# GemsLab/H2GCN

Measured on AMD Instinct MI355X. Metric: aggregated edges/sec (1+2-hop SpMM), higher is better.
Workload: dtype f32

## Files before the change

### h2gcn_amd/_capi.py

```python
from __future__ import annotations

import ctypes as C
import os
from pathlib import Path

ABI_VERSION = 5
MAX_HOPS = 8

OK = 0
ERR_INVALID_ARGUMENT = -1
ERR_HIP = -2
ERR_OUT_OF_MEMORY = -3
ERR_BAD_INDEX = -4
ERR_NO_TRANSPOSE = -5
ERR_INTERNAL = -6
ERR_EXCHANGE_TIMEOUT = -7

METRICS_MAX_SETS = 4
XCHG_BLOB_BYTES = 192
XCHG_COPY_ENGINE = 0
XCHG_COPY_KERNEL = 1

DTYPE_F32 = 0
DTYPE_BF16 = 1

PLAN_BUILD_TRANSPOSE = 0x1
PLAN_SKIP_VALIDATION = 0x2
PLAN_HOST_TRANSPOSE = 0x4
PLAN_KEEP_PERMUTATION = 0x8
PLAN_SYMMETRIC_PATTERN = 0x10

EXPORTED_SYMBOLS = (
    "h2gcn_abi_version",
    "h2gcn_last_error",
    "h2gcn_device_count",
    "h2gcn_plan_create",
    "h2gcn_plan_destroy",
    "h2gcn_plan_info",
    "h2gcn_plan_set_values",
    "h2gcn_plan_transpose_sharing",
    "h2gcn_plan_row_constant",
    "h2gcn_plan_device_bytes",
    "h2gcn_spmm_hops_f32",
    "h2gcn_spmm_hops_T_f32",
    "h2gcn_plan_schedule",
    "h2gcn_plan_segment_classes",
    "h2gcn_spmm_workspace_bytes",
    "h2gcn_spmm_hops_opts_f32",
    "h2gcn_spmm_hops_T_opts_f32",
    "h2gcn_spmm_hops_bf16",
    "h2gcn_spmm_hops_T_bf16",
    "h2gcn_sddmm_hops_f32",
    "h2gcn_sddmm_hops_bf16",
    "h2gcn_row_softmax_hops_f32",
    "h2gcn_row_softmax_backward_hops_f32",
    "h2gcn_edge_scores_hops_f32",
    "h2gcn_edge_scores_backward_hops_f32",
    "h2gcn_sddmm_hops_heads_f32",
    "h2gcn_row_softmax_hops_heads_f32",
    "h2gcn_row_softmax_backward_hops_heads_f32",
    "h2gcn_edge_scores_hops_heads_f32",
    "h2gcn_edge_scores_backward_hops_heads_f32",
    "h2gcn_spmm_hops_values_f32",
    "h2gcn_spmm_hops_T_values_f32",
    "h2gcn_ring_scratch_bytes",
    "h2gcn_ring_count",
    "h2gcn_ring_fill",
    "h2gcn_ring_count_rows",
    "h2gcn_ring_fill_rows",
    "h2gcn_hop_normalize",
    "h2gcn_hop_normalize_rows",
    "h2gcn_dropout_dense_small_rows",
    "h2gcn_dropout_dense_workspace_bytes",
    "h2gcn_dropout_dense_f32",
# ... 93 lines not shown
        C.POINTER(C.c_void_p), C.POINTER(C.c_void_p), C.POINTER(C.c_void_p),
        C.POINTER(PlanOpts), C.c_void_p, C.POINTER(C.c_void_p),
    ]
    L.h2gcn_plan_destroy.restype = None
    L.h2gcn_plan_destroy.argtypes = [C.c_void_p]
    L.h2gcn_plan_set_values.restype = C.c_int
    L.h2gcn_plan_set_values.argtypes = [C.c_void_p, C.c_int, C.c_void_p, C.c_void_p]
    L.h2gcn_plan_info.restype = C.c_int
    L.h2gcn_plan_info.argtypes = [
        C.c_void_p, C.c_int, C.POINTER(C.c_int64), C.POINTER(C.c_int64), C.POINTER(C.c_int64),
        C.POINTER(C.c_int64), C.POINTER(C.c_int32),
    ]
    L.h2gcn_spmm_hops_f32.restype = C.c_int
    L.h2gcn_spmm_hops_f32.argtypes = [
        C.c_void_p, C.c_uint32, C.c_void_p, C.c_int64, C.c_int32, C.c_void_p, C.c_int64, C.c_int64, C.c_void_p,
    ]
    L.h2gcn_spmm_hops_T_f32.restype = C.c_int
    L.h2gcn_spmm_hops_T_f32.argtypes = [
        C.c_void_p, C.c_uint32, C.c_void_p, C.c_int64, C.c_int64, C.c_int32, C.c_void_p, C.c_int64, C.c_void_p,
    ]
    L.h2gcn_plan_schedule.restype = C.c_int
    L.h2gcn_plan_schedule.argtypes = [C.c_void_p, C.c_uint32, C.c_int, C.c_int64, C.c_int32] + [C.POINTER(C.c_int32)] * 4
    if hasattr(L, "h2gcn_plan_segment_classes"):
        L.h2gcn_plan_segment_classes.restype = C.c_int
        L.h2gcn_plan_segment_classes.argtypes = [C.c_void_p, C.c_uint32, C.c_int, C.c_int64, C.c_int32] + [C.POINTER(C.c_int64)] * 3
    if hasattr(L, "h2gcn_plan_transpose_sharing"):
        L.h2gcn_plan_transpose_sharing.restype = C.c_int
        L.h2gcn_plan_transpose_sharing.argtypes = [C.c_void_p, C.c_int]
        L.h2gcn_plan_device_bytes.restype = C.c_size_t
        L.h2gcn_plan_device_bytes.argtypes = [C.c_void_p]
    if hasattr(L, "h2gcn_plan_row_constant"):
        L.h2gcn_plan_row_constant.restype = C.c_int
        L.h2gcn_plan_row_constant.argtypes = [C.c_void_p, C.c_int]
    L.h2gcn_spmm_workspace_bytes.restype = C.c_size_t
    L.h2gcn_spmm_workspace_bytes.argtypes = [C.c_void_p, C.c_uint32, C.c_int, C.c_void_p, C.c_int64, C.c_int64, C.c_int32]
    L.h2gcn_spmm_hops_opts_f32.restype = C.c_int
    L.h2gcn_spmm_hops_opts_f32.argtypes = [
        C.c_void_p, C.c_uint32, C.c_void_p, C.c_int64, C.c_int32, C.c_void_p, C.c_int64, C.c_int64,
        C.POINTER(LaunchOpts), C.c_void_p,
    ]
    L.h2gcn_spmm_hops_T_opts_f32.restype = C.c_int
    L.h2gcn_spmm_hops_T_opts_f32.argtypes = [
        C.c_void_p, C.c_uint32, C.c_void_p, C.c_int64, C.c_int64, C.c_int32, C.c_void_p, C.c_int64,
        C.POINTER(LaunchOpts), C.c_void_p,
    ]
    if hasattr(L, "h2gcn_spmm_hops_bf16"):
        L.h2gcn_spmm_hops_bf16.restype = C.c_int
        L.h2gcn_spmm_hops_bf16.argtypes = [
            C.c_void_p, C.c_uint32, C.c_void_p, C.c_int64, C.c_int32, C.c_int, C.c_void_p, C.c_int64, C.c_int64,
            C.POINTER(LaunchOpts), C.c_void_p,
        ]
        L.h2gcn_spmm_hops_T_bf16.restype = C.c_int
        L.h2gcn_spmm_hops_T_bf16.argtypes = [
            C.c_void_p, C.c_uint32, C.c_void_p, C.c_int64, C.c_int64, C.c_int32, C.c_int, C.c_void_p, C.c_int64,
            C.POINTER(LaunchOpts), C.c_void_p,
        ]
    if hasattr(L, "h2gcn_sddmm_hops_f32"):
        sddmm_args = [C.c_void_p, C.c_uint32, C.c_void_p, C.c_int64, C.c_int64, C.c_void_p, C.c_int64, C.c_int32,
                      C.POINTER(C.c_void_p), C.c_void_p]
        L.h2gcn_sddmm_hops_f32.restype = C.c_int
        L.h2gcn_sddmm_hops_f32.argtypes = sddmm_args
        L.h2gcn_sddmm_hops_bf16.restype = C.c_int
        L.h2gcn_sddmm_hops_bf16.argtypes = list(sddmm_args)
    if hasattr(L, "h2gcn_row_softmax_hops_f32"):
        L.h2gcn_row_softmax_hops_f32.restype = C.c_int
        L.h2gcn_row_softmax_hops_f32.argtypes = [C.c_void_p, C.c_uint32, C.POINTER(C.c_void_p), C.POINTER(C.c_void_p), C.c_void_p]
# ... 142 lines not shown
```

### h2gcn_amd/csrc/h2gcn_capi.hip

```cpp
#include <hip/hip_runtime.h>

#include <algorithm>
#include <cstdarg>
#include <cstdlib>
#include <cstdio>
#include <cstring>
#include <deque>
#include <map>
#include <mutex>
#include <memory>
#include <new>
#include <string>
#include <vector>

#include "h2gcn_hip.h"
#include "spmm_kernels.hip.h"

#include "capi_internal.h"

namespace h2gcn {

thread_local std::string g_last_error;

int fail(h2gcn_status st, const char* fmt, ...) {
// ... 11 lines not shown
namespace {

using h2gcn::fail;
using h2gcn::g_last_error;

struct DeviceBuf {
    void* p = nullptr;
    ~DeviceBuf() {
        if (p) (void)hipFree(p);
    }
    DeviceBuf() = default;
    DeviceBuf(DeviceBuf&& o) noexcept : p(o.p) { o.p = nullptr; }
    DeviceBuf(const DeviceBuf&) = delete;
    DeviceBuf& operator=(const DeviceBuf&) = delete;
};

struct HopOperand {
    const int64_t* rowptr = nullptr;
    const int32_t* colidx = nullptr;
    const float* vals = nullptr;
    int64_t nnz = 0;
    std::vector<int64_t> long_rows;
    std::vector<uint8_t> len8;
    int64_t n_short = 0, nnz_short = 0;
    int64_t nnz_long = 0;
    const uint32_t* perm = nullptr;
};

struct LongList {
    DeviceBuf dev;
    int n = 0;
    LongList() = default;
    LongList(LongList&&) noexcept = default;
};

struct ClassLists {
    DeviceBuf short_dev, med_dev;
    int64_t n_short = 0, nnz_short = 0, n_med = 0;
    bool built = false;
    ClassLists() = default;
    ClassLists(ClassLists&&) noexcept = default;
};

}

struct h2gcn_plan {
    int n_hops = 0;
    int64_t n_rows = 0, n_cols = 0;
    int long_threshold = 256;
    int rows_per_wave = 4;
    int variant = 0;
    int slice_cols = 0;
    bool has_transpose = false;
    int device = 0;
    std::vector<HopOperand> fwd;
    std::vector<HopOperand> adj;
    std::deque<DeviceBuf> owned;
    std::vector<int> sharing;
    size_t transpose_bytes = 0;
    std::vector<DeviceBuf> rowval;
    std::vector<char> row_const;
    mutable std::mutex mu;
    mutable std::map<uint64_t, LongList> long_cache;
    mutable std::map<uint64_t, ClassLists> class_cache;
    int short_max = -1;
    double short_min_frac = 0.05;
};

namespace h2gcn {
__global__ void check_colidx_kernel(const int32_t* __restrict__ colidx, int64_t nnz, int64_t n_cols, int* flag) {
    int bad = 0;
    for (int64_t i = (int64_t)blockIdx.x * blockDim.x + threadIdx.x; i < nnz; i += (int64_t)gridDim.x * blockDim.x) {
        const int32_t c = colidx[i];
        bad |= (c < 0) | ((int64_t)c >= n_cols);
    }
    if (bad) atomicOr(flag, 1);
}

__global__ void row_values_kernel(const int64_t* __restrict__ rowptr, const float* __restrict__ vals, int64_t n_rows,
                                  float* __restrict__ rowval, int* flag) {
    const int lane = threadIdx.x & (kWave - 1);
    const int64_t n_waves = ((int64_t)gridDim.x * blockDim.x) / kWave;
    const uint32_t* v = reinterpret_cast<const uint32_t*>(vals);
    int bad = 0;
    for (int64_t r = ((int64_t)blockIdx.x * blockDim.x + threadIdx.x) / kWave; r < n_rows; r += n_waves) {
        const int64_t b = rowptr[r], e = rowptr[r + 1];
        const uint32_t first = b < e ? v[b] : 0u;
        for (int64_t i = b + lane; i < e; i += kWave) bad |= v[i] != first;
        if (lane == 0) reinterpret_cast<uint32_t*>(rowval)[r] = first;
    }
    if (bad) atomicOr(flag, 1);
}

extern template void launch_in_tile_short_rows<32, false, float, float>(const LaunchParams&, const Schedule&, dim3, hipStream_t);
extern template void launch_in_tile_short_rows<16, false, float, float>(const LaunchParams&, const Schedule&, dim3, hipStream_t);
extern template void launch_in_tile_short_rows<32, true, float, float>(const LaunchParams&, const Schedule&, dim3, hipStream_t);
extern template void launch_in_tile_short_rows<16, true, float, float>(const LaunchParams&, const Schedule&, dim3, hipStream_t);
extern template void launch_spmm<false, bf16, float>(const LaunchParams&, const Schedule&, dim3, hipStream_t);
extern template void launch_spmm<false, bf16, bf16>(const LaunchParams&, const Schedule&, dim3, hipStream_t);
extern template void launch_spmm<true, bf16, float>(const LaunchParams&, const Schedule&, dim3, hipStream_t);
extern template void launch_spmm<true, bf16, bf16>(const LaunchParams&, const Schedule&, dim3, hipStream_t);

int transpose_csr_device(int64_t n_rows, int64_t n_cols, int64_t nnz, const int64_t* rowptr, const int32_t* colidx,
                         const float* vals, int64_t** t_rowptr_out, int32_t** t_colidx_out, float** t_vals_out,
                         uint32_t** perm_out_keep, hipStream_t stream, std::string* err);
void permute_values(const uint32_t* perm, const float* vals, int64_t nnz, float* t_vals, hipStream_t stream);
}

namespace {

using h2gcn::HopCsr;
using h2gcn::LaunchParams;
using h2gcn::Schedule;

int transpose_csr_host(int64_t n_rows, int64_t n_cols, const std::vector<int64_t>& rowptr,
                       const std::vector<int32_t>& colidx, const std::vector<float>& vals,
                       std::vector<int64_t>& t_rowptr, std::vector<int32_t>& t_colidx, std::vector<float>& t_vals) {
    const int64_t nnz = rowptr[n_rows];
    t_rowptr.assign(n_cols + 1, 0);
    t_colidx.resize(nnz);
    t_vals.resize(nnz);
    for (int64_t i = 0; i < nnz; ++i) t_rowptr[colidx[i] + 1]++;
    for (int64_t c = 0; c < n_cols; ++c) t_rowptr[c + 1] += t_rowptr[c];
    std::vector<int64_t> cursor(t_rowptr.begin(), t_rowptr.end() - 1);
// ... 139 lines not shown
    auto it = plan->long_cache.find(key);
    if (it == plan->long_cache.end()) {
        const std::vector<HopOperand>& ops = adjoint ? plan->adj : plan->fwd;
        std::vector<int64_t> host;
        int s = 0;
        if (!adjoint) {
            for (int k = 0; k < plan->n_hops; ++k) {
                if (!(mask & (1u << k))) continue;
                for (int64_t r : ops[k].long_rows) host.push_back((r << 4) | s);
                ++s;
            }
        } else {
            for (int k = 0; k < plan->n_hops; ++k) {
                if (!(mask & (1u << k))) continue;
                host.insert(host.end(), ops[k].long_rows.begin(), ops[k].long_rows.end());
            }
            std::sort(host.begin(), host.end());
            host.erase(std::unique(host.begin(), host.end()), host.end());
        }
        LongList fresh;
        fresh.n = (int)host.size();
        if (fresh.n > 0 && t_stream_capturing) return refuse_build_while_capturing("long-segment list");
        if (fresh.n > 0) {
            H2GCN_HIP_TRY(hipMalloc(&fresh.dev.p, host.size() * sizeof(int64_t)));
            H2GCN_HIP_TRY(hipMemcpy(fresh.dev.p, host.data(), host.size() * sizeof(int64_t), hipMemcpyHostToDevice));
        }
        it = plan->long_cache.emplace(key, std::move(fresh)).first;
    }
    *dev_out = (const int64_t*)it->second.dev.p;
    *n_out = it->second.n;
    return H2GCN_OK;
}

constexpr int64_t kWavesToFill = 12288;

bool aligned16(const void* p) { return (reinterpret_cast<uintptr_t>(p) & 15u) == 0; }

int pick_slice_cols(int d, int64_t n_src_rows, int forced, double avg_segment_nnz, bool rows_line_aligned = false) {
    if (forced > 0) return forced;
    if (d < 64) return 64;
    static const int widths[] = {256, 128, 64};
    for (int w : widths) {
        if (d % w != 0) continue;
        const double slice_bytes = (double)n_src_rows * w * 4.0;
        if (w > 64 && avg_segment_nnz >= 16.0 && slice_bytes > 768.0 * 1024 * 1024 && d % (w / 2) == 0) continue;
        return w;
    }
    if (rows_line_aligned && d % 4 == 0 && avg_segment_nnz >= 16.0 && (double)n_src_rows * d * 4.0 >= 512.0 * 1024 * 1024) {
        return 64;
    }
    if (d > 256) {
        const bool beyond = avg_segment_nnz >= 16.0 && (double)n_src_rows * 256 * 4.0 > 768.0 * 1024 * 1024;
        return beyond ? 128 : 256;
    }
    int w = 64;
    while (w < d) w *= 2;
    return w;
}

struct LaunchShape {
    bool adjoint;
    int n_sel;
    int64_t nnz_sel;
    int64_t n_out, n_src;
    double avg;
    int64_t ld_src;
// ... 90 lines not shown
            n_listed += sh.short_count[s];
            n_med += sh.med_count[s];
            longest = std::max(longest, sh.short_count[s]);
        }
        static const int env_mpw = getenv("H2GCN_MED_PER_WAVE") ? atoi(getenv("H2GCN_MED_PER_WAVE")) : 0;
        static const int env_spw = getenv("H2GCN_SHORT_PER_WAVE") ? atoi(getenv("H2GCN_SHORT_PER_WAVE")) : 0;
        static const int env_major = getenv("H2GCN_SHORT_HOP_MAJOR") ? atoi(getenv("H2GCN_SHORT_HOP_MAJOR")) : -1;
        const int mpw_max = adjoint ? std::max(1, std::min(4, kWave / p.n_sel)) : 8;
        p.med_per_wave = (int)std::max<int64_t>(1, std::min<int64_t>(n_med / kWavesToFill, mpw_max));
        if (env_mpw >= 1 && env_mpw * p.n_sel <= kWave) p.med_per_wave = env_mpw;
        p.short_per_wave = 4;
        while (p.short_per_wave < 64 && n_listed / (2 * p.short_per_wave) >= kWavesToFill) p.short_per_wave *= 2;
        if (env_spw >= 4 && env_spw <= 64 && env_spw % 4 == 0) p.short_per_wave = env_spw;
        p.short_hop_major = env_major >= 0 ? env_major : 0;
        int64_t sblocks = 0, mblocks = 0;
        const int64_t s_per_block = (int64_t)kWavesPerBlock * p.short_per_wave;
        for (int s = 0; s < sh.n_short_lists; ++s) {
            p.short_list[s] = sh.short_list[s];
            p.short_count[s] = sh.short_count[s];
            sblocks += (sh.short_count[s] + s_per_block - 1) / s_per_block;
            p.short_end[s] = sblocks;
            p.med_list[s] = sh.med_list[s];
            p.med_count[s] = sh.med_count[s];
            const int64_t per_block = (int64_t)kWavesPerBlock * p.med_per_wave;
            mblocks += (sh.med_count[s] + per_block - 1) / per_block;
            p.med_end[s] = mblocks;
        }
        if (!adjoint && !p.short_hop_major) sblocks = (longest + s_per_block - 1) / s_per_block * sh.n_short_lists;
        p.short_groups = (sblocks + kNumXcd - 1) / kNumXcd;
        p.med_groups = (mblocks + kNumXcd - 1) / kNumXcd;
        p.short_max = plan->short_max;
        p.blocks_per_slice = (int64_t)p.n_long + (p.short_groups + p.med_groups) * kNumXcd;
    } else {
        p.blocks_per_slice = (int64_t)p.n_long + p.tiles_per_xcd * kNumXcd;
    }
    const int64_t n_blocks = p.blocks_per_slice * p.n_slices;
    if (n_blocks <= 0) return H2GCN_OK;
    if (n_blocks > 0x7fffffffLL) return fail(H2GCN_ERR_INVALID_ARGUMENT, "grid too large (%lld blocks)", (long long)n_blocks);
    const dim3 grid((unsigned)n_blocks);
    Schedule rv = sc;
    rv.rowval = !adjoint && !out_bf16 && sc.exact && sc.slice == 64 && !sc.scalar128 && !sc.pipe && !sc.shortrow && !sc.lists &&
                !sc.gen && p.n_sel <= kRingHops;
    for (int k = 0, s = 0; rv.rowval && k < plan->n_hops; ++k) {
        if (!(mask & (1u << k))) continue;
        if (plan->row_const[(size_t)k] && plan->rowval[(size_t)k].p) p.rowval[s++] = (const float*)plan->rowval[(size_t)k].p;
        else rv.rowval = false;
    }
    if (!src_bf16 && adjoint) launch_spmm<true, float, float>(p, rv, grid, stream);
    else if (!src_bf16) launch_spmm<false, float, float>(p, rv, grid, stream);
    else if (out_bf16 && adjoint) launch_spmm<true, bf16, bf16>(p, rv, grid, stream);
    else if (out_bf16) launch_spmm<false, bf16, bf16>(p, rv, grid, stream);
    else if (adjoint) launch_spmm<true, bf16, float>(p, rv, grid, stream);
    else launch_spmm<false, bf16, float>(p, rv, grid, stream);
    H2GCN_HIP_TRY(hipGetLastError());
    return H2GCN_OK;
}

void use_scratch(LaunchParams& p, const LaunchShape& sh, int rs, int64_t ld_src_hop, void* workspace, hipStream_t stream,
                 bool* off32) {
    const int n_hop = sh.adjoint ? sh.n_sel : 1;
    const int n_slices = (sh.d + rs - 1) / rs;
    const bool vec4 = sh.d % 4 == 0;
    const int64_t total = sh.n_src * (int64_t)n_slices * n_hop * (rs / (vec4 ? 4 : 1));
    const unsigned blocks = (unsigned)std::min<int64_t>((total + 255) / 256, 256 * 64);
    if (vec4)
        hipLaunchKernelGGL(h2gcn::repack_slice_major_kernel<true>, dim3(blocks), dim3(256), 0, stream, (const float*)p.src, sh.ld_src,
                           ld_src_hop, n_hop, sh.n_src, sh.d, n_slices, rs, (float*)workspace);
// ... 257 lines not shown
            }
            plan->has_transpose = true;
        }
        {
            DeviceBuf rc_flag;
            H2GCN_HIP_TRY(hipMalloc(&rc_flag.p, (size_t)n_hops * sizeof(int)));
            H2GCN_HIP_TRY(hipMemsetAsync(rc_flag.p, 0, (size_t)n_hops * sizeof(int), stream));
            for (int k = 0; k < n_hops; ++k) {
                const HopOperand& op = plan->fwd[k];
                H2GCN_HIP_TRY(hipMalloc(&plan->rowval[k].p, (size_t)std::max<int64_t>(n_rows, 1) * sizeof(float)));
                if (n_rows == 0) continue;
                const unsigned blocks = (unsigned)std::min<int64_t>((n_rows + h2gcn::kWavesPerBlock - 1) / h2gcn::kWavesPerBlock, 8192);
                hipLaunchKernelGGL(h2gcn::row_values_kernel, dim3(blocks), dim3(h2gcn::kBlock), 0, stream, op.rowptr, op.vals, n_rows,
                                   (float*)plan->rowval[k].p, (int*)rc_flag.p + k);
                H2GCN_HIP_TRY(hipGetLastError());
            }
            std::vector<int> h_rc((size_t)n_hops, 0);
            H2GCN_HIP_TRY(hipMemcpyAsync(h_rc.data(), rc_flag.p, h_rc.size() * sizeof(int), hipMemcpyDeviceToHost, stream));
            H2GCN_HIP_TRY(hipStreamSynchronize(stream));
            for (int k = 0; k < n_hops; ++k) {
                plan->row_const[k] = h_rc[k] ? 0 : 1;
                if (!plan->row_const[k]) {
                    (void)hipFree(plan->rowval[k].p);
                    plan->rowval[k].p = nullptr;
                }
            }
        }
        {
            const uint32_t all = n_hops >= 32 ? 0xffffffffu : ((1u << n_hops) - 1u);
            const int64_t* unused_p = nullptr;
            int unused_n = 0;
            int st = get_long_list(plan.get(), false, all, &unused_p, &unused_n);
            if (st == H2GCN_OK && plan->has_transpose) st = get_long_list(plan.get(), true, all, &unused_p, &unused_n);
            if (st != H2GCN_OK) return st;
            auto mixed = [&](const LaunchShape& sh_) {
                return plan->variant == 6 || (plan->variant == 0 && sh_.short_frac >= plan->short_min_frac &&
                                              (sh_.avg >= 16.0 || sh_.n_out < 4 * kWavesToFill));
            };
            LaunchShape sh_f = shape_of(plan.get(), all, false);
            if ((st = fill_short(plan.get(), all, false, sh_f)) != H2GCN_OK) return st;
            if (mixed(sh_f) && (st = fill_short(plan.get(), all, false, sh_f, true)) != H2GCN_OK) return st;
            if (plan->has_transpose) {
                LaunchShape sh_a = shape_of(plan.get(), all, true);
                if ((st = fill_short(plan.get(), all, true, sh_a)) != H2GCN_OK) return st;
                if (mixed(sh_a) && (st = fill_short(plan.get(), all, true, sh_a, true)) != H2GCN_OK) return st;
            }
        }
        *out_plan = plan.release();
        return H2GCN_OK;
    } catch (const std::bad_alloc&) {
        return fail(H2GCN_ERR_OUT_OF_MEMORY, "host allocation failed in plan_create");
    } catch (...) {
        return fail(H2GCN_ERR_INTERNAL, "unexpected exception in plan_create");
    }
}

void h2gcn_plan_destroy(h2gcn_plan_t* plan) { delete plan; }

int h2gcn_plan_set_values(h2gcn_plan_t* plan, int hop, const float* vals_dev, void* stream_v) {
    if (!plan) return fail(H2GCN_ERR_INVALID_ARGUMENT, "plan is NULL");
    if (hop < 0 || hop >= plan->n_hops) return fail(H2GCN_ERR_INVALID_ARGUMENT, "hop %d outside 0..%d", hop, plan->n_hops - 1);
    HopOperand& f = plan->fwd[hop];
    if (f.nnz > 0 && !vals_dev) return fail(H2GCN_ERR_INVALID_ARGUMENT, "vals is NULL");
    int st = check_device(plan);
    if (st != H2GCN_OK) return st;
    if (plan->has_transpose) {
// ... 8 lines not shown
    if (plan->rowval[(size_t)hop].p) {
        hipStreamCaptureStatus cs = hipStreamCaptureStatusNone;
        if (hipStreamIsCapturing((hipStream_t)stream_v, &cs) != hipSuccess) (void)hipGetLastError();
        else if (cs == hipStreamCaptureStatusNone) {
            (void)hipFree(plan->rowval[(size_t)hop].p);
            plan->rowval[(size_t)hop].p = nullptr;
        }
    }
    return H2GCN_OK;
}

int h2gcn_plan_info(const h2gcn_plan_t* plan, int hop, int64_t* n_rows, int64_t* n_cols, int64_t* nnz,
                    int64_t* n_long_segments, int32_t* has_transpose) {
    if (!plan) return fail(H2GCN_ERR_INVALID_ARGUMENT, "plan is NULL");
    if (hop < 0 || hop >= plan->n_hops) return fail(H2GCN_ERR_INVALID_ARGUMENT, "hop %d outside 0..%d", hop, plan->n_hops - 1);
    if (n_rows) *n_rows = plan->n_rows;
    if (n_cols) *n_cols = plan->n_cols;
    if (nnz) *nnz = plan->fwd[hop].nnz;
    if (n_long_segments) *n_long_segments = (int64_t)plan->fwd[hop].long_rows.size();
    if (has_transpose) *has_transpose = plan->has_transpose ? 1 : 0;
    return H2GCN_OK;
}

int h2gcn_plan_transpose_sharing(const h2gcn_plan_t* plan, int hop) {
    if (!plan) return fail(H2GCN_ERR_INVALID_ARGUMENT, "plan is NULL");
    if (hop < 0 || hop >= plan->n_hops) return fail(H2GCN_ERR_INVALID_ARGUMENT, "hop %d outside 0..%d", hop, plan->n_hops - 1);
    return plan->sharing[(size_t)hop];
}

int h2gcn_plan_row_constant(const h2gcn_plan_t* plan, int hop) {
    if (!plan) return fail(H2GCN_ERR_INVALID_ARGUMENT, "plan is NULL");
    if (hop < 0 || hop >= plan->n_hops) return fail(H2GCN_ERR_INVALID_ARGUMENT, "hop %d outside 0..%d", hop, plan->n_hops - 1);
    return plan->row_const[(size_t)hop] ? 1 : 0;
}

size_t h2gcn_plan_device_bytes(const h2gcn_plan_t* plan) {
    if (!plan) return 0;
    std::lock_guard<std::mutex> lock(plan->mu);
    size_t bytes = plan->transpose_bytes;
    for (const DeviceBuf& rv : plan->rowval)
        if (rv.p) bytes += (size_t)std::max<int64_t>(plan->n_rows, 1) * sizeof(float);
    for (const auto& kv : plan->long_cache) bytes += (size_t)kv.second.n * sizeof(int64_t);
    for (const auto& kv : plan->class_cache)
        if (kv.second.built) bytes += (size_t)(kv.second.n_short + kv.second.n_med) * sizeof(int32_t);
    return bytes;
}

namespace {
int fill_short(const h2gcn_plan* plan, uint32_t mask, bool adjoint, LaunchShape& sh, bool build_lists) {
    sh.n_short_lists = 0;
    sh.short_frac = sh.short_nnz_frac = 0.0;
    if (plan->short_max < 0 || sh.n_out <= 0 || sh.n_sel <= 0) return H2GCN_OK;
    int64_t n = 0, nnz = 0;
    const ClassLists* cl = nullptr;
    if (!adjoint) {
        int s = 0;
        for (int k = 0; k < plan->n_hops; ++k) {
            if (!(mask & (1u << k))) continue;
            int st = get_class_lists(plan, false, k, 0, build_lists, &cl);
            if (st != H2GCN_OK) return st;
            if (!cl) return H2GCN_OK;
            sh.short_list[s] = (const int32_t*)cl->short_dev.p;
            sh.short_count[s] = cl->n_short;
            sh.med_list[s] = (const int32_t*)cl->med_dev.p;
            sh.med_count[s] = cl->n_med;
            n += cl->n_short;
// ... 167 lines not shown
        if (adjoint && (src.ld_row < d || src.ld_hop < 0)) return fail(H2GCN_ERR_INVALID_ARGUMENT, "bad gradient strides");
        if (!adjoint && sh.n_sel > 1 && dst.ld_hop < d)
            return fail(H2GCN_ERR_INVALID_ARGUMENT, "ldy_hop = %lld < d = %d: hop outputs would overlap", (long long)dst.ld_hop, d);
        CaptureScope capture_scope((hipStream_t)stream_v);
        LaunchParams p;
        memset(&p, 0, sizeof(p));
        const std::vector<HopOperand>& ops = adjoint ? plan->adj : plan->fwd;
        int s = 0;
        for (int k = 0; k < plan->n_hops; ++k) {
            if (!(mask & (1u << k))) continue;
            const HopOperand& op = ops[k];
            p.hop[s] = HopCsr{op.rowptr, op.colidx, op.vals};
            p.src_hop_off[s] = (int64_t)s * src.ld_hop;
            p.dst_hop_off[s] = (int64_t)s * dst.ld_hop;
            ++s;
        }
        p.n_sel = s;
        p.d = d;
        p.d_src = d;
        p.n_rows = sh.n_out;
        p.src = src.ptr;
        p.ld_src = src.ld_row;
        p.dst = const_cast<void*>(dst.ptr);
        p.ld_dst = dst.ld_row;
        p.bias = lo.bias_dev;
        p.relu = (lo.flags & H2GCN_LAUNCH_RELU) ? 1 : 0;
        p.accumulate = (lo.flags & H2GCN_LAUNCH_ACCUMULATE) ? 1 : 0;
        st = get_long_list(plan, adjoint, mask, &p.long_list, &p.n_long);
        if (st != H2GCN_OK) return st;
        p.long_threshold = plan->long_threshold;
        p.rows_per_wave = plan->rows_per_wave;
        const int64_t rows_per_tile = (int64_t)p.rows_per_wave * kWavesPerBlock;
        p.n_tiles = (p.n_rows + rows_per_tile - 1) / rows_per_tile;
        p.tiles_per_xcd = (p.n_tiles + kNumXcd - 1) / kNumXcd;
        const int64_t esz = src.bf16 ? 2 : 4;
        bool off32 = ((double)(sh.n_src > 0 ? sh.n_src - 1 : 0) * (double)src.ld_row + (double)(s - 1) * (double)src.ld_hop + d) *
                     (double)esz < 4294967296.0;
        int scratch = (!src.bf16 && lo.workspace_dev && aligned16(lo.workspace_dev)) ? scratch_slice_cols(plan, sh) : 0;
        if (scratch > 0 && lo.workspace_bytes >= scratch_bytes(sh, scratch)) {
            use_scratch(p, sh, scratch, src.ld_hop, lo.workspace_dev, (hipStream_t)stream_v, &off32);
            H2GCN_HIP_TRY(hipGetLastError());
        } else {
            scratch = 0;
        }
        const bool gen = d % 4 != 0 || p.bias != nullptr || p.relu != 0 || p.accumulate != 0;
        Schedule sc;
        if ((st = decide(plan, mask, sh, scratch, gen, sc)) != H2GCN_OK) return st;
        static const bool force_off64 = getenv("H2GCN_FORCE_OFF64") != nullptr;
        sc.off32 = off32 && !force_off64;
        return launch(p, plan, mask, sh, sc, adjoint, src.bf16, dst.bf16, (hipStream_t)stream_v);
    } catch (...) {
        return fail(H2GCN_ERR_INTERNAL, "unexpected exception in spmm_hops_%s",
                    adjoint ? (src.bf16 ? "T_bf16" : "T_f32") : (src.bf16 ? "bf16" : "opts_f32"));
    }
}
}

extern "C++" {
namespace h2gcn {
int pattern_view(const h2gcn_plan* plan, uint32_t hop_mask, PatternView* out) {
    if (!plan) return fail(H2GCN_ERR_INVALID_ARGUMENT, "plan is NULL");
    memset(out, 0, sizeof(*out));
    const int st = resolve_mask(plan, hop_mask, &out->mask);
    if (st != H2GCN_OK) return st;
    out->n_rows = plan->n_rows;
    out->n_cols = plan->n_cols;
    out->long_threshold = plan->long_threshold;
// ... 84 lines not shown
```

### h2gcn_amd/csrc/spmm_kernels.hip.h

```cpp
#pragma once

#include <hip/hip_runtime.h>
#include <stdint.h>

#include <type_traits>

#include "h2gcn_hip.h"

namespace h2gcn {

constexpr int kWave = 64;
constexpr int kWavesPerBlock = 4;
constexpr int kBlock = kWave * kWavesPerBlock;
constexpr int kNumXcd = 8;
constexpr int kMaxRowsPerWave = 7;
#ifndef H2GCN_MIN_WAVES
#define H2GCN_MIN_WAVES 6
#endif
constexpr int kMinWavesPerSimd = H2GCN_MIN_WAVES;
#ifndef H2GCN_SHORT_MIN_WAVES
#define H2GCN_SHORT_MIN_WAVES 4
#endif
#ifndef H2GCN_SHORT_FB4_MIN_WAVES
#define H2GCN_SHORT_FB4_MIN_WAVES 7
// ... 39 lines not shown
    int d;
    int d_src;
    int64_t n_rows;
    const void* src;
    int64_t ld_src;
    int64_t src_slice_stride;
    void* dst;
    int64_t ld_dst;
    const int64_t* long_list;
    int n_long;
    int long_threshold;
    int rows_per_wave;
    int64_t n_tiles;
    int64_t tiles_per_xcd;
    int n_slices;
    int slice_cols;
    int64_t blocks_per_slice;
    const float* bias;
    int relu;
    int accumulate;
    const int32_t* short_list[H2GCN_MAX_HOPS];
    int64_t short_count[H2GCN_MAX_HOPS];
    int64_t short_end[H2GCN_MAX_HOPS];
    int64_t short_groups;
    int short_max;
    int short_per_wave;
    int short_hop_major;
    const int32_t* med_list[H2GCN_MAX_HOPS];
    int64_t med_count[H2GCN_MAX_HOPS];
    int64_t med_end[H2GCN_MAX_HOPS];
    int64_t med_groups;
    int med_per_wave;
    const float* rowval[H2GCN_MAX_HOPS];
};

template <int VEC>
struct VecT;
template <>
struct VecT<1> {
    using type = float;
};
template <>
struct VecT<2> {
    typedef float type __attribute__((ext_vector_type(2), aligned(4)));
};
template <>
struct VecT<4> {
    typedef float type __attribute__((ext_vector_type(4), aligned(4)));
};

struct bf16 {
    uint16_t bits;
};

template <typename TS, int VEC>
struct LoadT {
    using type = typename VecT<VEC>::type;
};
template <>
struct LoadT<bf16, 4> {
    typedef uint32_t type __attribute__((ext_vector_type(2), aligned(4)));
};
template <>
struct LoadT<bf16, 2> {
    using type = uint32_t;
};
// ... 930 lines not shown
    const bool heavy = VEC == 4 && (LISTS ? (SUM && (!OFF32 || LPR >= 32)) || (!OFF32 && LPR >= 32) : !OFF32 || (PIPE && LPR == 32));
    if (heavy) return H2GCN_OFF64_HEAVY_MIN_WAVES - bf16_less;
    return (LPR >= 32 ? H2GCN_WIDE_MIN_WAVES : kMinWavesPerSimd) - bf16_less;
}

template <int VEC, int LPR, bool EXACT, bool SUM, bool OFF32, bool PIPE = false, bool SHORT = false, bool EPI = false, int FB = 8, bool LISTS = false,
          typename TS = float, typename TD = float, bool ROWVAL = false>
__global__ __launch_bounds__(kBlock, (min_waves_per_simd<VEC, LPR, EXACT, SUM, OFF32, PIPE, SHORT, EPI, FB, LISTS, TS>())) void spmm_hops_kernel(const LaunchParams p) {
    static_assert(!LISTS || (EXACT && !SHORT && !PIPE && (LPR == 16 || LPR == 32)), "list-driven launches exist for 64- and 128-column slices");
    static_assert(EXACT || LPR == kWave, "column-tiled path uses the whole wave per row");
    static_assert(!ROWVAL || (uses_index_window<LPR, EXACT, PIPE, SHORT, EPI, LISTS>() && !SUM), "row values: forward walk on the index window");
    __shared__ float partial[kWavesPerBlock][kMaxTileCols];
    using off_t = typename std::conditional<OFF32, uint32_t, int64_t>::type;
    constexpr int NP = Tree<LPR>::NP;
    constexpr int kMainB = LISTS ? FB : (LPR >= 32 ? H2GCN_WIDE_MAXB : H2GCN_MAIN_MAXB);

    const int lane = threadIdx.x & (kWave - 1);
    const int wave = wave_uniform(threadIdx.x >> 6);
    const int li = lane % LPR;
    const int g = lane / LPR;
    const int n_sel = p.n_sel;

    const int64_t bid = blockIdx.x;
    const int slice = EXACT ? (int)(bid / p.blocks_per_slice) : 0;
    const int64_t b = EXACT ? bid - (int64_t)slice * p.blocks_per_slice : bid;
    const int col_begin = EXACT ? slice * (VEC * LPR) : 0;
    const int col_end = EXACT ? col_begin + VEC * LPR : p.d;
    const int64_t src_col_begin = EXACT ? (int64_t)slice * p.src_slice_stride : 0;
    const int lcol = col_begin + li * VEC;
    const int ecol = EXACT ? ((lcol + VEC <= p.d_src) ? lcol : p.d_src - VEC) : lcol;
    const off_t lane_off0 = (off_t)((ecol - col_begin + VEC) * (int)sizeof(TS));
    constexpr int kBias = EXACT ? VEC : 0;

    if (b < p.n_long) {
        const int64_t entry = p.long_list[b];
        const int64_t row = SUM ? entry : (entry >> 4);
        const int s_first = SUM ? 0 : (int)(entry & 15);
        const int s_last = SUM ? n_sel : s_first + 1;
        for (int col0 = col_begin; col0 < col_end; col0 += VEC * LPR) {
            const bool lane_active = EXACT || (col0 + li * VEC < p.d);
            float acc[NP][VEC];
            zero_acc<VEC, NP>(acc);
            for (int s = s_first; s < s_last; ++s) {
                const HopCsr& h = p.hop[s];
                const int64_t sb = h.rowptr[row], se = h.rowptr[row + 1];
                const GatherAddr<OFF32> addr{reinterpret_cast<const char*>(src_ptr<TS>(p.src) + p.src_hop_off[s] + src_col_begin + (col0 - col_begin) - kBias),
                                             EXACT ? lane_off0 : (off_t)(li * VEC * (int)sizeof(TS)), (off_t)(p.ld_src * sizeof(TS))};
                if constexpr (ROWVAL)
                    accumulate_segment<TS, VEC, LPR, !EXACT, OFF32, kMainB, true>(h.colidx, nullptr, sb, se, wave, kWavesPerBlock, addr, lane,
                                                                              lane_active, acc, p.rowval[s][row]);
                else
                    accumulate_segment<TS, VEC, LPR, !EXACT, OFF32, kMainB>(h.colidx, h.vals, sb, se, wave, kWavesPerBlock, addr, lane,
                                                                            lane_active, acc);
            }
            float tot[VEC];
            fold_tree<VEC, LPR, NP>(acc, tot);
            if (g == 0) {
                const int rel = EXACT ? ecol - col_begin : li * VEC;
                if (!EXACT || lcol < p.d_src) {
#pragma unroll
                    for (int i = 0; i < VEC; ++i)
                        if (rel + i >= 0) partial[wave][rel + i] = tot[i];
                }
            }
            __syncthreads();
            const int c = threadIdx.x;
            if (c < VEC * LPR && col0 + c < p.d) {
                float t = partial[0][c];
#pragma unroll
                for (int w = 1; w < kWavesPerBlock; ++w) t += partial[w][c];
                const int64_t off = row * p.ld_dst + (SUM ? 0 : p.dst_hop_off[s_first]) + col0 + c;
                if constexpr (EPI) {
                    if constexpr (std::is_same<TD, float>::value)
                        if (p.accumulate) t += dst_ptr<float>(p.dst)[off];
                    if (p.bias) t += p.bias[col0 + c];
                    if (p.relu) t = relu_keep_nan(t);
                }
                store_one<TD>(dst_ptr<TD>(p.dst) + off, t);
            }
            if (!EXACT) __syncthreads();
        }
        return;
    }

    const int64_t tb = b - p.n_long;
    int64_t tile;
    if constexpr (LISTS) {
        __shared__ uint64_t s_seg[kWavesPerBlock][kShortSumHops][kWave];
        __shared__ int32_t s_row[kWavesPerBlock][kWave];
        const int64_t q = tb >> 3;
        const int i8 = (int)(tb & 7);
        const int64_t n_groups = p.short_groups + p.med_groups;
        const int64_t s_before = (q * p.short_groups) / n_groups;
        if (((q + 1) * p.short_groups) / n_groups > s_before)
            short_list_blocks<TS, TD, VEC, LPR, SUM, OFF32, EPI, H2GCN_SHORT_PREFETCH>(p, s_before * kNumXcd + i8, lane, wave, (int64_t)lane_off0,
                                                                               src_col_begin, lcol, ecol, s_seg, s_row);
        else
            medium_list_blocks<TS, TD, VEC, LPR, SUM, OFF32, EPI, FB>(p, (q - s_before) * kNumXcd + i8, lane, wave, (int64_t)lane_off0,
                                                              src_col_begin, lcol, ecol);
        return;
    } else {
        tile = (tb % kNumXcd) * p.tiles_per_xcd + tb / kNumXcd;
    }
    if (tile >= p.n_tiles) return;
    const int rpw = p.rows_per_wave;
    const int64_t row0 = (tile * kWavesPerBlock + wave) * rpw;
    if (row0 >= p.n_rows) return;
    const int64_t rows_here_l = p.n_rows - row0;
    const int rows_here = rows_here_l < rpw ? (int)rows_here_l : rpw;

    int64_t rp = 0;
    float rv = 0.f;
    {
        const int hs = lane / (rpw + 1), r = lane % (rpw + 1);
        if (hs < n_sel && r <= rows_here) rp = p.hop[hs].rowptr[row0 + r];
        if constexpr (ROWVAL)
            if (hs < n_sel && r < rows_here) rv = p.rowval[hs][row0 + r];
    }
    const int rp_lo = (int)(rp & 0xffffffff), rp_hi = (int)(rp >> 32);
    auto seg_bound = [&](int l) -> int64_t {
        return ((int64_t)__builtin_amdgcn_readlane(rp_hi, l) << 32) | (uint32_t)__builtin_amdgcn_readlane(rp_lo, l);
    };

    if constexpr (SHORT && EXACT && (kWave / LPR == 2 || kWave / LPR == 4)) {
        in_tile_short_rows<TS, TD, VEC, LPR, SUM, OFF32, EPI, FB>(p, lane, rpw, row0, rows_here, rp_lo, rp_hi, (int64_t)lane_off0, src_col_begin, lcol, ecol);
        return;
    }
    if constexpr (uses_index_window<LPR, EXACT, PIPE, SHORT, EPI, LISTS>()) {
        __shared__ uint32_t ring[kWavesPerBlock][kRingHops][(ROWVAL ? 1 : 2) * kRingCap];
        bool fits = n_sel <= kRingHops;
#pragma unroll
        for (int s = 0; s < kRingHops; ++s)
            if (s < n_sel && seg_bound(s * (rpw + 1) + rows_here) - seg_bound(s * (rpw + 1)) > kRingMaxRange) fits = false;
        if (fits) {
            window_tile_walk<TS, TD, VEC, LPR, SUM, OFF32, EPI, kMainB, ROWVAL>(p, lane, rpw, row0, rows_here, rp, (int64_t)lane_off0, src_col_begin, lcol,
// ... 265 lines not shown
```

### h2gcn_amd/hops.py

```python
from __future__ import annotations

import ctypes as C
from typing import Iterable, Optional, Sequence

import torch

from . import _capi


def _require(cond: bool, msg: str) -> None:
    if not cond:
        raise ValueError(msg)


def _bf16_layout(name: str, t: torch.Tensor, d: int, strides) -> None:
    _require(d % 2 == 0, f"bf16 {name}: the feature width d must be even (got {d})")
    _require(t.data_ptr() % 4 == 0, f"bf16 {name}: the base address must be 4-byte aligned")
    for st in strides:
        _require(st % 2 == 0, f"bf16 {name}: row / hop strides must be even (got {tuple(strides)} elements)")


def _bf16_symbols() -> None:
    _require(_capi.has("h2gcn_spmm_hops_bf16"), f"{_capi.library_path()} predates the bf16 launches (ABI 5)")

# ... 161 lines not shown
    def device_bytes(self) -> int:
        if not _capi.has("h2gcn_plan_device_bytes"):
            raise RuntimeError(f"{_capi.library_path()} predates h2gcn_plan_device_bytes")
        return int(_capi.lib().h2gcn_plan_device_bytes(self._handle))

    def schedule(self, d: int, ld_src: Optional[int] = None, hops=None, adjoint: bool = False) -> dict:
        L = _capi.lib()
        sc, ns, pf, cp = C.c_int32(), C.c_int32(), C.c_int32(), C.c_int32()
        ld = int(ld_src) if ld_src is not None else (self.n_selected(hops) * d if adjoint else d)
        _capi.check(L.h2gcn_plan_schedule(self._handle, self._mask(hops), 1 if adjoint else 0, ld, int(d),
                                          C.byref(sc), C.byref(ns), C.byref(pf), C.byref(cp)))
        return dict(slice_cols=sc.value, n_slices=ns.value,
                    segment_walk={0: "wave per segment", 1: "wave per segment + index prefetch",
                                  2: "lane group per segment (short rows)",
                                  3: "lane group per segment (binned short segments) + wave per segment"}[pf.value],
                    scratch_copy=bool(cp.value) and self.use_workspace)

    def segment_classes(self, d: int, ld_src: Optional[int] = None, hops=None, adjoint: bool = False) -> dict:
        L = _capi.lib()
        if not _capi.has("h2gcn_plan_segment_classes"):
            raise RuntimeError(f"{_capi.library_path()} predates h2gcn_plan_segment_classes (ABI 4)")
        h_sel = self.n_selected(hops)
        seg, nnz, listed = (C.c_int64 * (3 * h_sel))(), (C.c_int64 * (3 * h_sel))(), C.c_int64()
        ld = int(ld_src) if ld_src is not None else (h_sel * d if adjoint else d)
        _capi.check(L.h2gcn_plan_segment_classes(self._handle, self._mask(hops), 1 if adjoint else 0, ld, int(d), seg, nnz, C.byref(listed)))
        sel = self._selected(hops)
        short_walk = ("lane group per segment (binned list)" if listed.value > 0 else
                      "lane group per segment (rounds of consecutive short rows)" if listed.value < 0 else "wave per segment")
        per_hop = [dict(hop=sel[s], segments=dict(short=seg[3 * s], medium=seg[3 * s + 1], long=seg[3 * s + 2]),
                        nonzeros=dict(short=nnz[3 * s], medium=nnz[3 * s + 1], long=nnz[3 * s + 2])) for s in range(h_sel)]
        return dict(per_hop=per_hop, listed=listed.value,
                    walks=dict(short=short_walk, medium="wave per segment", long="workgroup per segment (4 waves, LDS-staged)"))

    def _mask(self, hops) -> int:
        if hops is None:
            return 0
        mask = 0
        for h in hops:
            _require(0 <= int(h) < self.n_hops, f"hop index {h} outside 0..{self.n_hops - 1}")
            mask |= 1 << int(h)
        _require(mask != 0, "empty hop selection")
        return mask

    def _selected(self, hops) -> list:
        return list(range(self.n_hops)) if hops is None else sorted({int(h) for h in hops})

    def n_selected(self, hops) -> int:
        return self.n_hops if hops is None else bin(self._mask(hops)).count("1")

    def spmm(self, x: torch.Tensor, hops=None, out: Optional[torch.Tensor] = None, bias: Optional[torch.Tensor] = None,
             relu: bool = False, out_dtype: Optional[torch.dtype] = None) -> torch.Tensor:
        _require(x.dim() == 2, f"inputs must be [n_cols, d], got shape {tuple(x.shape)}")
        _require(x.dtype in (torch.float32, torch.bfloat16), f"inputs must be float32 or bfloat16, got {x.dtype}")
        _require(x.device == self.device, f"inputs on {x.device}, plan on {self.device}")
        _require(x.shape[0] == self.n_cols, f"inputs have {x.shape[0]} rows, hop matrices have {self.n_cols} columns")
        d = int(x.shape[1])
        _require(d >= 1, "inputs need at least one column")
        bf16 = x.dtype == torch.bfloat16
        if out_dtype is None:
            out_dtype = out.dtype if out is not None else x.dtype
        _require(out_dtype in (torch.float32, torch.bfloat16), f"outputs must be float32 or bfloat16, got {out_dtype}")
        _require(bf16 or out_dtype == torch.float32, "float32 inputs give float32 outputs (float32 -> bfloat16 is not supported)")
        if x.stride(1) != 1:
            x = x.contiguous()
        h_sel = self.n_selected(hops)
        if out is None:
# ... 483 lines not shown
```

### include/h2gcn_hip.h

```cpp
#ifndef H2GCN_HIP_H_
#define H2GCN_HIP_H_

#include <stddef.h>
#include <stdint.h>

#ifdef __cplusplus
extern "C" {
#endif

#define H2GCN_ABI_VERSION 5
#define H2GCN_MAX_HOPS 8

typedef enum h2gcn_status {
    H2GCN_OK = 0,
    H2GCN_ERR_INVALID_ARGUMENT = -1,
    H2GCN_ERR_HIP = -2,
    H2GCN_ERR_OUT_OF_MEMORY = -3,
    H2GCN_ERR_BAD_INDEX = -4,
    H2GCN_ERR_NO_TRANSPOSE = -5,
    H2GCN_ERR_INTERNAL = -6,
    H2GCN_ERR_EXCHANGE_TIMEOUT = -7
} h2gcn_status;

#define H2GCN_PLAN_BUILD_TRANSPOSE 0x1u
// ... 7 lines not shown
typedef struct h2gcn_plan_opts {
    uint32_t struct_size;
    uint32_t flags;
    int32_t long_row_threshold;
    int32_t rows_per_wave;
    int32_t variant;
    int32_t slice_cols;
    int32_t reserved[2];
} h2gcn_plan_opts;

typedef struct h2gcn_plan h2gcn_plan_t;

int h2gcn_abi_version(void);

const char* h2gcn_last_error(void);

int h2gcn_device_count(void);

int h2gcn_plan_create(int n_hops, int64_t n_rows, int64_t n_cols,
                      const int64_t* const* rowptr_dev, const int32_t* const* colidx_dev,
                      const float* const* vals_dev, const h2gcn_plan_opts* opts, void* stream,
                      h2gcn_plan_t** out_plan);

void h2gcn_plan_destroy(h2gcn_plan_t* plan);

int h2gcn_plan_set_values(h2gcn_plan_t* plan, int hop, const float* vals_dev, void* stream);

int h2gcn_plan_info(const h2gcn_plan_t* plan, int hop, int64_t* n_rows, int64_t* n_cols, int64_t* nnz,
                    int64_t* n_long_segments, int32_t* has_transpose);

int h2gcn_plan_transpose_sharing(const h2gcn_plan_t* plan, int hop);

int h2gcn_plan_row_constant(const h2gcn_plan_t* plan, int hop);

size_t h2gcn_plan_device_bytes(const h2gcn_plan_t* plan);

int h2gcn_plan_schedule(const h2gcn_plan_t* plan, uint32_t hop_mask, int adjoint, int64_t ld_src, int32_t d,
                        int32_t* slice_cols, int32_t* n_slices, int32_t* segment_walk, int32_t* scratch_copy);

int h2gcn_plan_segment_classes(const h2gcn_plan_t* plan, uint32_t hop_mask, int adjoint, int64_t ld_src, int32_t d,
                               int64_t* segments, int64_t* nonzeros, int64_t* listed);

int h2gcn_spmm_hops_f32(const h2gcn_plan_t* plan, uint32_t hop_mask, const float* X_dev, int64_t ldx,
                        int32_t d, float* Y_dev, int64_t ldy_row, int64_t ldy_hop, void* stream);

#define H2GCN_LAUNCH_RELU 0x1u
#define H2GCN_LAUNCH_ACCUMULATE 0x2u
typedef struct h2gcn_launch_opts {
    uint32_t struct_size;
    uint32_t flags;
    void* workspace_dev;
    size_t workspace_bytes;
    const float* bias_dev;
} h2gcn_launch_opts;
size_t h2gcn_spmm_workspace_bytes(const h2gcn_plan_t* plan, uint32_t hop_mask, int adjoint, const float* src_dev,
                                  int64_t ld_src, int64_t ld_src_hop, int32_t d);
int h2gcn_spmm_hops_opts_f32(const h2gcn_plan_t* plan, uint32_t hop_mask, const float* X_dev, int64_t ldx,
                             int32_t d, float* Y_dev, int64_t ldy_row, int64_t ldy_hop,
                             const h2gcn_launch_opts* opts, void* stream);

int h2gcn_spmm_hops_T_f32(const h2gcn_plan_t* plan, uint32_t hop_mask, const float* dY_dev, int64_t ldg_row,
                          int64_t ldg_hop, int32_t d, float* dX_dev, int64_t ldx, void* stream);
int h2gcn_spmm_hops_T_opts_f32(const h2gcn_plan_t* plan, uint32_t hop_mask, const float* dY_dev, int64_t ldg_row,
                               int64_t ldg_hop, int32_t d, float* dX_dev, int64_t ldx,
                               const h2gcn_launch_opts* opts, void* stream);

// ... 157 lines not shown
```

Before: 14.03 billion.

## Balance SpMM tile ranges across XCDs by nonzero count

```diff
diff --git a/h2gcn_amd/_capi.py b/h2gcn_amd/_capi.py
--- a/h2gcn_amd/_capi.py
+++ b/h2gcn_amd/_capi.py
@@ -40,6 +40,7 @@
     "h2gcn_plan_set_values",
     "h2gcn_plan_transpose_sharing",
     "h2gcn_plan_row_constant",
+    "h2gcn_plan_xcd_balance",
     "h2gcn_plan_device_bytes",
     "h2gcn_spmm_hops_f32",
     "h2gcn_spmm_hops_T_f32",
@@ -199,6 +200,9 @@
     if hasattr(L, "h2gcn_plan_row_constant"):
         L.h2gcn_plan_row_constant.restype = C.c_int
         L.h2gcn_plan_row_constant.argtypes = [C.c_void_p, C.c_int]
+    if hasattr(L, "h2gcn_plan_xcd_balance"):
+        L.h2gcn_plan_xcd_balance.restype = C.c_int
+        L.h2gcn_plan_xcd_balance.argtypes = [C.c_void_p, C.c_uint32, C.c_int, C.POINTER(C.c_int64), C.POINTER(C.c_int64)]
     L.h2gcn_spmm_workspace_bytes.restype = C.c_size_t
     L.h2gcn_spmm_workspace_bytes.argtypes = [C.c_void_p, C.c_uint32, C.c_int, C.c_void_p, C.c_int64, C.c_int64, C.c_int32]
     L.h2gcn_spmm_hops_opts_f32.restype = C.c_int
diff --git a/h2gcn_amd/csrc/h2gcn_capi.hip b/h2gcn_amd/csrc/h2gcn_capi.hip
--- a/h2gcn_amd/csrc/h2gcn_capi.hip
+++ b/h2gcn_amd/csrc/h2gcn_capi.hip
@@ -67,6 +67,12 @@
     int n = 0;
     LongList() = default;
     LongList(LongList&&) noexcept = default;
+};
+
+struct XcdSplit {
+    int64_t begin[h2gcn::kNumXcd + 1] = {};
+    int64_t nnz[h2gcn::kNumXcd] = {};
+    int64_t max_tiles = 0;
 };
 
 struct ClassLists {
@@ -97,6 +103,7 @@
     std::vector<char> row_const;
     mutable std::mutex mu;
     mutable std::map<uint64_t, LongList> long_cache;
+    mutable std::map<uint64_t, XcdSplit> xcd_cache;
     mutable std::map<uint64_t, ClassLists> class_cache;
     int short_max = -1;
     double short_min_frac = 0.05;
@@ -125,6 +132,46 @@
         if (lane == 0) reinterpret_cast<uint32_t*>(rowval)[r] = first;
     }
     if (bad) atomicOr(flag, 1);
+}
+
+struct XcdWorkArgs {
+    const int64_t* rowptr[H2GCN_MAX_HOPS];
+    int n_sel;
+    int sum;
+    int long_threshold;
+    int rows_per_tile;
+    int64_t n_rows, n_tiles;
+    const int64_t* long_list;
+    int n_long;
+};
+
+__global__ void xcd_work_kernel(const XcdWorkArgs a, int64_t* __restrict__ out) {
+    const int64_t i = (int64_t)blockIdx.x * blockDim.x + threadIdx.x;
+    if (i < a.n_tiles) {
+        const int64_t r0 = i * a.rows_per_tile;
+        const int64_t r1 = r0 + a.rows_per_tile < a.n_rows ? r0 + a.rows_per_tile : a.n_rows;
+        int64_t z = 0;
+        for (int64_t r = r0; r < r1; ++r) {
+            int64_t row = 0;
+            bool any_long = false;
+            for (int s = 0; s < a.n_sel; ++s) {
+                const int64_t len = a.rowptr[s][r + 1] - a.rowptr[s][r];
+                if (len >= a.long_threshold) any_long = true;
+                else row += len;
+            }
+            if (!(a.sum && any_long)) z += row;
+        }
+        out[i] = z;
+    } else if (i < a.n_tiles + a.n_long) {
+        const int64_t entry = a.long_list[i - a.n_tiles];
+        const int64_t r = a.sum ? entry : (entry >> 4);
+        int64_t z = 0;
+        for (int s = a.sum ? 0 : (int)(entry & 15); s < a.n_sel; ++s) {
+            z += a.rowptr[s][r + 1] - a.rowptr[s][r];
+            if (!a.sum) break;
+        }
+        out[i] = z;
+    }
 }
 
 extern template void launch_in_tile_short_rows<32, false, float, float>(const LaunchParams&, const Schedule&, dim3, hipStream_t);
@@ -330,6 +377,74 @@
     return H2GCN_OK;
 }
 
+void choose_xcd_boundaries(const std::vector<int64_t>& tile_prefix, const int64_t* long_nnz, int n_long, XcdSplit& sp) {
+    constexpr int X = h2gcn::kNumXcd;
+    const int64_t n_tiles = (int64_t)tile_prefix.size() - 1;
+    int64_t long_of[X] = {};
+    for (int j = 0; j < n_long; ++j) long_of[j % X] += long_nnz[j];
+    int64_t total = tile_prefix[(size_t)n_tiles];
+    for (int x = 0; x < X; ++x) total += long_of[x];
+    int64_t long_so_far = 0;
+    sp.begin[0] = 0;
+    for (int x = 0; x + 1 < X; ++x) {
+        long_so_far += long_of[x];
+        const int64_t target = (int64_t)(((__int128)total * (x + 1)) / X) - long_so_far;
+        const auto first = tile_prefix.begin() + sp.begin[x];
+        int64_t e = std::lower_bound(first, tile_prefix.end(), target) - tile_prefix.begin();
+        if (e > n_tiles) e = n_tiles;
+        if (e > sp.begin[x] && target - tile_prefix[(size_t)e - 1] <= tile_prefix[(size_t)e] - target) --e;
+        sp.begin[x + 1] = e;
+    }
+    sp.begin[X] = n_tiles;
+    sp.max_tiles = 0;
+    for (int x = 0; x < X; ++x) {
+        sp.nnz[x] = long_of[x] + tile_prefix[(size_t)sp.begin[x + 1]] - tile_prefix[(size_t)sp.begin[x]];
+        sp.max_tiles = std::max(sp.max_tiles, sp.begin[x + 1] - sp.begin[x]);
+    }
+}
+
+int get_xcd_split(const h2gcn_plan* plan, bool adjoint, uint32_t mask, const XcdSplit** out) {
+    *out = nullptr;
+    const int64_t* long_list = nullptr;
+    int n_long = 0;
+    int st = get_long_list(plan, adjoint, mask, &long_list, &n_long);
+    if (st != H2GCN_OK) return st;
+    const uint64_t key = (uint64_t)mask | ((uint64_t)(adjoint ? 1 : 0) << 32);
+    std::lock_guard<std::mutex> lock(plan->mu);
+    auto it = plan->xcd_cache.find(key);
+    if (it == plan->xcd_cache.end()) {
+        if (t_stream_capturing) return refuse_build_while_capturing("XCD split");
+        const std::vector<HopOperand>& ops = adjoint ? plan->adj : plan->fwd;
+        h2gcn::XcdWorkArgs a;
+        memset(&a, 0, sizeof(a));
+        for (int k = 0; k < plan->n_hops; ++k)
+            if (mask & (1u << k)) a.rowptr[a.n_sel++] = ops[k].rowptr;
+        a.sum = adjoint ? 1 : 0;
+        a.long_threshold = plan->long_threshold;
+        a.rows_per_tile = plan->rows_per_wave * h2gcn::kWavesPerBlock;
+        a.n_rows = adjoint ? plan->n_cols : plan->n_rows;
+        a.n_tiles = (a.n_rows + a.rows_per_tile - 1) / a.rows_per_tile;
+        a.long_list = long_list;
+        a.n_long = n_long;
+        const int64_t n_items = a.n_tiles + n_long;
+        std::vector<int64_t> work((size_t)n_items + 1, 0);
+        if (n_items > 0) {
+            DeviceBuf dev;
+            H2GCN_HIP_TRY(hipMalloc(&dev.p, (size_t)n_items * sizeof(int64_t)));
+            hipLaunchKernelGGL(h2gcn::xcd_work_kernel, dim3((unsigned)((n_items + 255) / 256)), dim3(256), 0, (hipStream_t)0, a, (int64_t*)dev.p);
+            H2GCN_HIP_TRY(hipGetLastError());
+            H2GCN_HIP_TRY(hipMemcpy(work.data() + 1, dev.p, (size_t)n_items * sizeof(int64_t), hipMemcpyDeviceToHost));
+        }
+        for (int64_t t = 1; t <= a.n_tiles; ++t) work[(size_t)t] += work[(size_t)t - 1];
+        std::vector<int64_t> prefix(work.begin(), work.begin() + a.n_tiles + 1);
+        XcdSplit fresh;
+        choose_xcd_boundaries(prefix, work.data() + a.n_tiles + 1, n_long, fresh);
+        it = plan->xcd_cache.emplace(key, fresh).first;
+    }
+    *out = &it->second;
+    return H2GCN_OK;
+}
+
 constexpr int64_t kWavesToFill = 12288;
 
 bool aligned16(const void* p) { return (reinterpret_cast<uintptr_t>(p) & 15u) == 0; }
@@ -486,7 +601,15 @@
         p.short_max = plan->short_max;
         p.blocks_per_slice = (int64_t)p.n_long + (p.short_groups + p.med_groups) * kNumXcd;
     } else {
-        p.blocks_per_slice = (int64_t)p.n_long + p.tiles_per_xcd * kNumXcd;
+        const XcdSplit* sp = nullptr;
+        const int st = get_xcd_split(plan, adjoint, mask, &sp);
+        if (st != H2GCN_OK) return st;
+        if (sp->begin[kNumXcd] != p.n_tiles) return fail(H2GCN_ERR_INTERNAL, "XCD split covers %lld tiles, the launch has %lld",
+                                                         (long long)sp->begin[kNumXcd], (long long)p.n_tiles);
+        for (int x = 0; x <= kNumXcd; ++x) p.xcd_tile_begin[x] = sp->begin[x];
+        p.tiles_per_xcd = sp->max_tiles;
+        p.n_long_pad = (p.n_long + kNumXcd - 1) / kNumXcd * kNumXcd;
+        p.blocks_per_slice = (int64_t)p.n_long_pad + p.tiles_per_xcd * kNumXcd;
     }
     const int64_t n_blocks = p.blocks_per_slice * p.n_slices;
     if (n_blocks <= 0) return H2GCN_OK;
@@ -810,6 +933,9 @@
             int unused_n = 0;
             int st = get_long_list(plan.get(), false, all, &unused_p, &unused_n);
             if (st == H2GCN_OK && plan->has_transpose) st = get_long_list(plan.get(), true, all, &unused_p, &unused_n);
+            const XcdSplit* unused_sp = nullptr;
+            if (st == H2GCN_OK) st = get_xcd_split(plan.get(), false, all, &unused_sp);
+            if (st == H2GCN_OK && plan->has_transpose) st = get_xcd_split(plan.get(), true, all, &unused_sp);
             if (st != H2GCN_OK) return st;
             auto mixed = [&](const LaunchShape& sh_) {
                 return plan->variant == 6 || (plan->variant == 0 && sh_.short_frac >= plan->short_min_frac &&
@@ -884,6 +1010,20 @@
     if (!plan) return fail(H2GCN_ERR_INVALID_ARGUMENT, "plan is NULL");
     if (hop < 0 || hop >= plan->n_hops) return fail(H2GCN_ERR_INVALID_ARGUMENT, "hop %d outside 0..%d", hop, plan->n_hops - 1);
     return plan->row_const[(size_t)hop] ? 1 : 0;
+}
+
+int h2gcn_plan_xcd_balance(const h2gcn_plan_t* plan, uint32_t hop_mask, int adjoint, int64_t* tile_begin, int64_t* nnz) {
+    if (!plan) return fail(H2GCN_ERR_INVALID_ARGUMENT, "plan is NULL");
+    uint32_t mask = 0;
+    int st = resolve_mask(plan, hop_mask, &mask);
+    if (st != H2GCN_OK) return st;
+    if (adjoint && !plan->has_transpose) return fail(H2GCN_ERR_NO_TRANSPOSE, "plan was created without H2GCN_PLAN_BUILD_TRANSPOSE");
+    if ((st = check_device(plan)) != H2GCN_OK) return st;
+    const XcdSplit* sp = nullptr;
+    if ((st = get_xcd_split(plan, adjoint != 0, mask, &sp)) != H2GCN_OK) return st;
+    for (int x = 0; tile_begin && x <= h2gcn::kNumXcd; ++x) tile_begin[x] = sp->begin[x];
+    for (int x = 0; nnz && x < h2gcn::kNumXcd; ++x) nnz[x] = sp->nnz[x];
+    return H2GCN_OK;
 }
 
 size_t h2gcn_plan_device_bytes(const h2gcn_plan_t* plan) {
@@ -1117,7 +1257,6 @@
         p.rows_per_wave = plan->rows_per_wave;
         const int64_t rows_per_tile = (int64_t)p.rows_per_wave * kWavesPerBlock;
         p.n_tiles = (p.n_rows + rows_per_tile - 1) / rows_per_tile;
-        p.tiles_per_xcd = (p.n_tiles + kNumXcd - 1) / kNumXcd;
         const int64_t esz = src.bf16 ? 2 : 4;
         bool off32 = ((double)(sh.n_src > 0 ? sh.n_src - 1 : 0) * (double)src.ld_row + (double)(s - 1) * (double)src.ld_hop + d) *
                      (double)esz < 4294967296.0;
diff --git a/h2gcn_amd/csrc/spmm_kernels.hip.h b/h2gcn_amd/csrc/spmm_kernels.hip.h
--- a/h2gcn_amd/csrc/spmm_kernels.hip.h
+++ b/h2gcn_amd/csrc/spmm_kernels.hip.h
@@ -95,6 +95,8 @@
     int64_t med_groups;
     int med_per_wave;
     const float* rowval[H2GCN_MAX_HOPS];
+    int64_t xcd_tile_begin[kNumXcd + 1];
+    int n_long_pad;
 };
 
 template <int VEC>
@@ -1091,7 +1093,10 @@
     const off_t lane_off0 = (off_t)((ecol - col_begin + VEC) * (int)sizeof(TS));
     constexpr int kBias = EXACT ? VEC : 0;
 
-    if (b < p.n_long) {
+    const int n_long_blocks = LISTS ? p.n_long : p.n_long_pad;
+    if (b < n_long_blocks) {
+        if constexpr (!LISTS)
+            if (b >= p.n_long) return;
         const int64_t entry = p.long_list[b];
         const int64_t row = SUM ? entry : (entry >> 4);
         const int s_first = SUM ? 0 : (int)(entry & 15);
@@ -1142,7 +1147,7 @@
         return;
     }
 
-    const int64_t tb = b - p.n_long;
+    const int64_t tb = b - n_long_blocks;
     int64_t tile;
     if constexpr (LISTS) {
         __shared__ uint64_t s_seg[kWavesPerBlock][kShortSumHops][kWave];
@@ -1159,7 +1164,9 @@
                                                               src_col_begin, lcol, ecol);
         return;
     } else {
-        tile = (tb % kNumXcd) * p.tiles_per_xcd + tb / kNumXcd;
+        const int x = (int)(tb % kNumXcd);
+        tile = p.xcd_tile_begin[x] + tb / kNumXcd;
+        if (tile >= p.xcd_tile_begin[x + 1]) return;
     }
     if (tile >= p.n_tiles) return;
     const int rpw = p.rows_per_wave;
diff --git a/h2gcn_amd/hops.py b/h2gcn_amd/hops.py
--- a/h2gcn_amd/hops.py
+++ b/h2gcn_amd/hops.py
@@ -217,6 +217,13 @@
         return dict(per_hop=per_hop, listed=listed.value,
                     walks=dict(short=short_walk, medium="wave per segment", long="workgroup per segment (4 waves, LDS-staged)"))
 
+    def xcd_balance(self, hops=None, adjoint: bool = False) -> dict:
+        if not _capi.has("h2gcn_plan_xcd_balance"):
+            raise RuntimeError(f"{_capi.library_path()} predates h2gcn_plan_xcd_balance")
+        begin, nnz = (C.c_int64 * 9)(), (C.c_int64 * 8)()
+        _capi.check(_capi.lib().h2gcn_plan_xcd_balance(self._handle, self._mask(hops), 1 if adjoint else 0, begin, nnz))
+        return dict(tile_begin=list(begin), nnz=list(nnz))
+
     def _mask(self, hops) -> int:
         if hops is None:
             return 0
diff --git a/include/h2gcn_hip.h b/include/h2gcn_hip.h
--- a/include/h2gcn_hip.h
+++ b/include/h2gcn_hip.h
@@ -63,6 +63,8 @@
 int h2gcn_plan_transpose_sharing(const h2gcn_plan_t* plan, int hop);
 
 int h2gcn_plan_row_constant(const h2gcn_plan_t* plan, int hop);
+
+int h2gcn_plan_xcd_balance(const h2gcn_plan_t* plan, uint32_t hop_mask, int adjoint, int64_t* tile_begin, int64_t* nnz);
 
 size_t h2gcn_plan_device_bytes(const h2gcn_plan_t* plan);
 
```

After: 14.07 billion (median of 5 runs). About the same (+0.3%).
